# TSultanov/cfd-demo

Hardware: AMD Instinct MI355X
Metric: cell-updates/s (Poisson iter) + ms/timestep, 4096² grid, 1/2/4/8 GPU (higher is better)
Workload: dtype f32

## Files before the change

### cfd-demo_amd/cfdamd/__init__.py

```python
from __future__ import annotations

import ctypes as C
import enum
from dataclasses import dataclass
from typing import List, Optional

import numpy as np

from . import _lib
from ._lib import (CFD_ENONFINITE, CfdError, CfdGrid, CfdParams, CfdResiduals, CfdState, check,
                   load)

__all__ = [
    "VelocityScheme", "InletProfile", "PressureSolver", "BoundaryKind", "Cylinder", "Grid",
    "SimulationParams", "Residuals", "SimSnapshot", "Model", "SimulationControlHandle",
    "CfdError", "default_grid", "cavity_grid", "rccl_unique_id", "device_count", "load", "LocalHub",
    "VisualizationMode", "CFD_ENONFINITE",
]


class VelocityScheme(enum.IntEnum):
    FirstOrder = 0
    SecondOrder = 1

# ... 385 lines not shown
        return {"state": int(s.value), "m0": int(a.value), "rm": int(b.value)}

    @property
    def comm_calls(self) -> int:
        n = C.c_uint64()
        check("cfd_get_comm_calls", load().cfd_get_comm_calls(self._hh(), C.byref(n)))
        return int(n.value)

    @property
    def recoveries(self) -> int:
        n = C.c_uint64()
        check("cfd_get_recoveries", load().cfd_get_recoveries(self._hh(), C.byref(n)))
        return int(n.value)

    @property
    def resident_solves(self) -> int:
        n = C.c_uint64()
        check("cfd_get_resident_solves", load().cfd_get_resident_solves(self._hh(), C.byref(n)))
        return int(n.value)

    @property
    def persist_blocks(self) -> int:
        n = C.c_int()
        check("cfd_get_persist_blocks", load().cfd_get_persist_blocks(self._hh(), C.byref(n)))
        return n.value

    @property
    def comm_size(self) -> int:
        n = C.c_int()
        check("cfd_get_comm_size", load().cfd_get_comm_size(self._hh(), C.byref(n)))
# ... 107 lines not shown
```

### cfd-demo_amd/cfdamd/_lib.py

```python
from __future__ import annotations

import ctypes as C
import os

PKG_DIR = os.path.dirname(os.path.abspath(__file__))
ROOT = os.path.dirname(PKG_DIR)
LIB_PATH = os.environ.get("CFD_LIB") or os.path.join(ROOT, "lib", "libcfd_amd.so")

EXPORTS = [
    "cfd_default_params", "cfd_default_grid", "cfd_create", "cfd_rccl_unique_id",
    "cfd_create_sharded", "cfd_local_hub_create", "cfd_local_hub_destroy",
    "cfd_create_sharded_local", "cfd_device_count", "cfd_get_comm_size", "cfd_get_slab", "cfd_update", "cfd_update_n", "cfd_piso_step",
    "cfd_pressure_solve", "cfd_run_phase", "cfd_set_params", "cfd_get_snapshot",
    "cfd_get_residuals", "cfd_get_state", "cfd_set_state", "cfd_get_masks", "cfd_synchronize",
    "cfd_profile_sweeps", "cfd_timing_begin", "cfd_timing_end", "cfd_timing_phases",
    "cfd_timing_phase_ms", "cfd_timing_exchange_ms", "cfd_get_halo_depth",
    "cfd_get_kernel_config", "cfd_get_jacobi_kernel", "cfd_get_persist_blocks", "cfd_get_persist_steals", "cfd_get_persist_sums", "cfd_get_sums_launches", "cfd_get_sums_bounds", "cfd_get_recoveries", "cfd_get_comm_calls", "cfd_get_resident_solves", "cfd_get_jacobi_geometry", "cfd_plan_slab", "cfd_plan_sweep", "cfd_plan_halo", "cfd_plan_block", "cfd_plan_overlap",
    "cfd_render", "cfd_derive_field", "cfd_last_error", "cfd_abi_version", "cfd_destroy",
    "cfd_get_config", "cfd_run_start", "cfd_run_stop", "cfd_run_pause", "cfd_run_resume",
    "cfd_run_set_params", "cfd_run_request_snapshot", "cfd_run_last_snapshot",
    "cfd_run_new_residuals", "cfd_run_status", "cfd_run_steps",
    "cfd_polygon_new", "cfd_polygon_new_rect", "cfd_polygon_new_regular", "cfd_polygon_add_hole",
    "cfd_polygon_contains_point", "cfd_polygon_intersects_aabb",
    "cfd_polygon_edges_intersect_aabb", "cfd_polygon_bounding_box",
    "cfd_polygon_bounding_square", "cfd_polygon_edges", "cfd_polygon_destroy",
    "cfd_geom_do_intersect", "cfd_geom_segment_intersection", "cfd_geom_intersect_quad_edge",
    "cfd_tesselate", "cfd_quadtree_size", "cfd_quadtree_nodes", "cfd_quadtree_destroy",
    "cfd_mesh_from_quadtree", "cfd_mesh_sizes", "cfd_mesh_cells", "cfd_mesh_neighbors",
    "cfd_mesh_intersections", "cfd_mesh_full_bounding_box", "cfd_mesh_build_ms",
    "cfd_mesh_destroy",
]

# ... 93 lines not shown
        "cfd_timing_phases": (i32, [vp, i32]),
        "cfd_timing_phase_ms": (i32, [vp, C.POINTER(C.c_double), C.POINTER(C.c_double)]),
        "cfd_timing_exchange_ms": (i32, [vp, C.POINTER(C.c_double), C.POINTER(C.c_uint64)]),
        "cfd_get_halo_depth": (i32, [vp]),
        "cfd_get_kernel_config": (i32, [vp, C.POINTER(i32), C.POINTER(i32)]),
        "cfd_get_jacobi_kernel": (i32, [vp, C.POINTER(i32), C.c_char_p, C.c_size_t]),
        "cfd_get_persist_blocks": (i32, [vp, C.POINTER(i32)]),
        "cfd_get_persist_steals": (i32, [vp, C.POINTER(C.c_uint64)]),
        "cfd_get_persist_sums": (i32, [vp, C.POINTER(C.c_uint64)]),
        "cfd_get_sums_launches": (i32, [vp, C.POINTER(C.c_uint64)]),
        "cfd_get_sums_bounds": (i32, [vp, C.POINTER(C.c_uint32), C.POINTER(C.c_uint32),
                                      C.POINTER(C.c_uint32)]),
        "cfd_get_recoveries": (i32, [vp, C.POINTER(C.c_uint64)]),
        "cfd_get_comm_calls": (i32, [vp, C.POINTER(C.c_uint64)]),
        "cfd_get_resident_solves": (i32, [vp, C.POINTER(C.c_uint64)]),
        "cfd_get_jacobi_geometry": (i32, [vp, i32, C.POINTER(i32), C.POINTER(i32), C.POINTER(i32),
                                          C.POINTER(i32)]),
        "cfd_plan_slab": (i32, [C.c_uint64, i32, i32, C.POINTER(C.c_uint64),
                                C.POINTER(C.c_uint64)]),
        "cfd_plan_sweep": (i32, [i32, i32, i32, i32, i32, i32, C.POINTER(i32), C.POINTER(i32),
                                 C.POINTER(i32)]),
        "cfd_plan_halo": (i32, [i32, i32, i32, i32, i32, C.POINTER(i32)]),
        "cfd_plan_overlap": (i32, [i32, i32, i32, i32, i32, i32, C.POINTER(i32)]),
        "cfd_plan_block": (i32, [i32, i32, i32, i32, i32, i32, i32, C.POINTER(i32),
                                 C.POINTER(i32), C.POINTER(i32), C.POINTER(i32)]),
        "cfd_render": (i32, [vp, i32, C.POINTER(C.c_uint8), FP]),
        "cfd_derive_field": (i32, [vp, i32, FP, FP]),
        "cfd_last_error": (C.c_char_p, []),
        "cfd_abi_version": (i32, []),
        "cfd_destroy": (None, [vp]),
# ... 57 lines not shown
```

### cfd-demo_amd/csrc/cfd_device.h

```cpp
#pragma once
#include "cfd_internal.h"

#include <algorithm>

namespace cfd {
namespace {

inline int cdiv(long a, long b) { return (int)((a + b - 1) / b); }


constexpr int kBlock = 256;
typedef unsigned int u32x4 __attribute__((ext_vector_type(4)));

__device__ __forceinline__ float dt_of(const Ctl *c, float dt_override) {
    return __builtin_isnan(dt_override) ? c->dt : dt_override;
}

__device__ __forceinline__ bool pass_off(const Ctl *c, int pass) {
    return pass >= 0 && c->go[pass] == 0;
}

__device__ __forceinline__ float wave_max(float m) {
#pragma unroll
    for (int o = 32; o > 0; o >>= 1) m = fmaxf(m, __shfl_xor(m, o, 64));
// ... 58 lines not shown
}

template <int SP>
__device__ __forceinline__ float sdiv(float x, float c, float r) {
    return SP ? x * r : x / c;
}

typedef float f2 __attribute__((ext_vector_type(2)));

template <int FAST>
__device__ __forceinline__ f2 fdiv2(f2 x, float c, float r) {
    if (FAST == 1) return x * r;
    return (f2){fdiv<FAST>(x.x, c, r), fdiv<FAST>(x.y, c, r)};
}

__device__ __forceinline__ void solve_finalize_body(const Geom &g, const Fields &f, int pass,
                                                    int iters, int check_break, int flips,
                                                    int exact_flips) {
    Ctl *c = f.ctl;
    __shared__ int go_s;
    const int k_lo = g.tol_enabled ? 0 : (iters > 0 ? iters - 1 : 0);
    const int wv = (int)threadIdx.x >> 6, nw = (int)blockDim.x >> 6;
    for (int k = k_lo + wv; k < iters; k += nw) {
        uint32_t *set = f.err_slots + (size_t)k * kResSlots * kResStride;
        const float v = read_max(set, c->err[k]);
        if ((threadIdx.x & 63) < kResSlots) set[(threadIdx.x & 63) * kResStride] = 0u;
        if ((threadIdx.x & 63) == 0) c->err[k] = __float_as_uint(v);
    }
    __syncthreads();
    if (threadIdx.x == 0) {
        const int go = pass < 0 ? 1 : c->go[pass];
        if (go) {
            int n = iters;
            if (g.tol_enabled && iters > 0) {
                n = 1;
                while (n < iters && !(__uint_as_float(c->err[n - 1]) < g.p_tol)) ++n;
            }
            const float res = n > 0 ? __uint_as_float(c->err[n - 1]) : 0.0f;
            c->cur = (c->cur + (exact_flips == 2 ? c->spec_launches
                                : (g.tol_enabled && !exact_flips) ? n : flips)) & 1;
            c->last_p = res;
            c->red[5] = __float_as_uint(res);
            c->n_exec_last = (uint32_t)n;
            c->sweeps_total += (uint64_t)n;
        }
        if (pass >= 0 && pass + 1 <= kMaxPasses)
            c->go[pass + 1] = (go && !(check_break && g.tol_enabled && c->last_p < g.p_tol)) ? 1 : 0;
        if (exact_flips >= 2) c->spec_stop = c->spec_redo = c->spec_launch = c->spec_launches = 0;
        c->sums_state = 0u;
        c->sums_m0 = 0u;
        go_s = go;
    }
    __syncthreads();
    if (go_s)
        for (int k = threadIdx.x; k < iters; k += blockDim.x) c->err[k] = 0u;
}

template <int FAST>
__device__ __forceinline__ float4 jacobi_row4(const float4 &B, const float4 &C, const float4 &T,
                                              const float4 &Rh, float L0, float R3, float dx_sq,
                                              float dy_sq, float denom, float r_dx_sq,
                                              float r_dy_sq, float r_denom) {
    const f2 c01 = {C.x, C.y}, c23 = {C.z, C.w};
    const f2 h01 = __builtin_shufflevector(c01, c01, 1, 0) + (f2){L0, C.z};
    const f2 h23 = __builtin_shufflevector(c23, c23, 1, 0) + (f2){C.y, R3};
    const f2 v01 = (f2){T.x, T.y} + (f2){B.x, B.y};
    const f2 v23 = (f2){T.z, T.w} + (f2){B.z, B.w};
    const f2 hz01 = fdiv2<FAST>(h01, dx_sq, r_dx_sq), hz23 = fdiv2<FAST>(h23, dx_sq, r_dx_sq);
    const f2 vt01 = fdiv2<FAST>(v01, dy_sq, r_dy_sq), vt23 = fdiv2<FAST>(v23, dy_sq, r_dy_sq);
    const f2 pu01 = fdiv2<FAST>(hz01 + vt01 - (f2){Rh.x, Rh.y}, denom, r_denom);
// ... 11 lines not shown
```

### cfd-demo_amd/csrc/cfd_internal.h

```cpp
#pragma once
#include <hip/hip_runtime.h>
#include <stdint.h>

#include "../../include/cfd.h"

namespace cfd {

constexpr int kGhostUV = 2;
constexpr float kSumsPLim = 0x1p122f, kSumsRLim = 0x1p112f;
constexpr int kMaxSweeps = 4096;
constexpr int kMaxPasses = 64;

constexpr int kResSlots = 32;
constexpr int kResStride = 16;
constexpr int kPersistFlagStride = 16;
constexpr int kPersistHeadLines = 21;
constexpr int kPersistBlockBits = 10;
static_assert((1 << kPersistBlockBits) > kMaxSweeps / 8, "persistent flag layout");
constexpr int kPersistMaxGroups = 16384;
constexpr size_t kPersistWords = (size_t)(kPersistMaxGroups + kPersistHeadLines) * kPersistFlagStride;
constexpr size_t kSlotWords = (size_t)(kMaxSweeps + 16) * kResSlots * kResStride + kPersistWords;

struct Ctl {
    float dt;
// ... 2 lines not shown
    float inlet;
    int32_t cur;
    uint32_t n_exec_last;
    float last_p;
    float res_u, res_v;
    uint32_t red[7];
    uint32_t nonfinite_step;
    uint32_t vis[2];
    uint32_t sums_state;
    uint64_t sweeps_total;
    int32_t spec_stop, spec_redo, spec_launch, spec_launches;
    uint32_t sums_launches;
    uint32_t sums_m0, sums_rm;
    int32_t go[kMaxPasses + 1];
    uint32_t err[kMaxSweeps];
};

struct Geom {
    int32_t nx, ny;
    int32_t j0, nyl;
    int32_t hg;
    float dx, dy, nu, ly;
    float target_inlet;
    int32_t scheme, profile, bc_kind;
    int32_t tol_enabled;
    float p_tol;
    int32_t jacobi_iters;
    float dx_sq, dy_sq, denom;
    float r_dx_sq, r_dy_sq, r_denom;
    int32_t fastdiv;
    int32_t tb_rows;
// ... 30 lines not shown
void launch_step_begin(const Geom &g, const Fields &f, int copy, hipStream_t s);
void launch_copy_star(const Geom &g, const Fields &f, int pass, hipStream_t s);
void launch_copy_star_div(const Geom &g, const Fields &f, int pass, float dt_override,
                          hipStream_t s);
void launch_u_predictor(const Geom &g, const Fields &f, float dt_override, hipStream_t s);
void launch_v_predictor(const Geom &g, const Fields &f, float dt_override, hipStream_t s);
void launch_predict(const Geom &g, const Fields &f, float dt_override, hipStream_t s);
bool predict_march_ok(const Geom &g, const Fields &f);
void launch_predict_march(const Geom &g, const Fields &f, float dt_override, hipStream_t s,
                          bool set_inlet = false, int row_lo = 0, int row_hi = -1);
void launch_divergence(const Geom &g, const Fields &f, int pass, float dt_override,
                       hipStream_t s);
void launch_jacobi_sweep(const Geom &g, const Fields &f, int pass, int it, int row_lo,
                         int row_hi, int res, hipStream_t s);
void launch_jacobi_block(const Geom &g, const Fields &f, int pass, int it, int par, int T,
                         int out_lo, int out_hi, int res, hipStream_t s);
bool launch_jacobi_persist(const Geom &g, const Fields &f, int pass, int par0, int nblk,
                           int out_lo, int out_hi, uint32_t epoch, int res_it, hipStream_t s);
void lds_geometry8(const Geom &g, int out_lo, int out_hi, bool persist, int *pad, int *occ, int *nwc,
                   int *nseg);
void launch_tb1(const Geom &g, const Fields &f, int T, int pass, int it, int par, int out_lo,
                int out_hi, uint32_t *res_slots, hipStream_t s);
void launch_pipe(const Geom &g, const Fields &f, int T, int pass, int it, int par, int out_lo,
                 int out_hi, uint32_t *res_slots, hipStream_t s);
bool launch_lds_persist8(const Geom &g, const Fields &f, int pass, int par0, int nblk, int out_lo,
                         int out_hi, uint32_t epoch, uint32_t *rs, hipStream_t s);
void launch_lds(const Geom &g, const Fields &f, int T, int pass, int it, int par, int out_lo,
                int out_hi, uint32_t *res_slots, hipStream_t s, int mode = 0, int lag = 0);
void launch_jacobi_spec(const Geom &g, const Fields &f, int pass, int it, int par, int T,
                        int out_lo, int out_hi, hipStream_t s, int lag = 0);
void launch_spec_check(const Geom &g, const Fields &f, int pass, int it, int T, int par,
// ... 45 lines not shown
void launch_mg_prolong_smooth5(const MgLevel &Cl, const float *e, const MgLevel &L, const float *src,
                               float *dst, const Ctl *ctl, int pass, hipStream_t s);
void launch_mg_smooth5_residual(const MgLevel &L, const float *src, float *dst, const Ctl *ctl,
                                int pass, hipStream_t s);
void launch_mg_residual(const MgLevel &L, const float *p, const Ctl *ctl, int pass, hipStream_t s);
void launch_mg_restrict(const MgLevel &F, const MgLevel &Cl, const Ctl *ctl, int pass, hipStream_t s);
void launch_mg_prolong_add(const MgLevel &Cl, const float *e, const MgLevel &F, float *p,
                           const Ctl *ctl, int pass, hipStream_t s);
void launch_mg_tail(const MgLevel *dev_levels, int s_level, int coarsest, float *a0, float *b0,
                    int fast, const Ctl *ctl, int pass, hipStream_t s);
void launch_mg_final_residual(const MgLevel &L, const float *p, uint32_t *slots, const Ctl *ctl,
                              int pass, hipStream_t s);
void launch_corrector(const Geom &g, const Fields &f, int pass, float dt_override,
                      hipStream_t s);
void launch_boundary(const Geom &g, const Fields &f, hipStream_t s);
void launch_correct_finish(const Geom &g, const Fields &f, float dt_override, hipStream_t s);
void launch_step_reduce(const Geom &g, const Fields &f, hipStream_t s);
void launch_publish_sums_m0(const Geom &g, const Fields &f, hipStream_t s);
bool correct_head_ok(const Geom &g, const Fields &f);
void launch_correct_head(const Geom &g, const Fields &f, int pass, float dt_override, bool has_next,
                         hipStream_t s);
void launch_step_finalize(const Geom &g, const Fields &f, hipStream_t s);
void launch_abort_to_red(const Fields &f, hipStream_t s);
void launch_abort_from_red(const Fields &f, hipStream_t s);

constexpr int kJacRowsPerWave = 16;
constexpr int kMaxTemporal = 8;
constexpr int kJacWavesPerBlock = 4;

}
```

### cfd-demo_amd/csrc/cfd_jacobi_lds.h

```cpp
#pragma once
#include <cmath>
#include <type_traits>

#include "cfd_device.h"

namespace cfd {
namespace {

constexpr int kLdsWaves = 4;
#ifndef CFD_LDS_SB
#define CFD_LDS_SB 0
#endif
#ifndef CFD_LDS_PD
#define CFD_LDS_PD 3
#endif
#ifndef CFD_LDS_DIAG
#define CFD_LDS_DIAG 0
#endif
#ifndef CFD_LDS_WPE
#define CFD_LDS_WPE 0
#endif
typedef unsigned int u32x2 __attribute__((ext_vector_type(2)));
#ifndef CFD_LDS_PRIO
#define CFD_LDS_PRIO 1
// ... 427 lines not shown
            ctl->spec_launch = lpar;
            ctl->spec_redo = j + 1 < T ? j + 1 : 0;
        }
    }
    return j;
}

template <int T, int FAST, int MODE>
__global__ __launch_bounds__(kLdsWaves * 64, lds_min_waves(MODE)) void k_jacobi_lds(
    Geom g, float *__restrict__ pa, float *__restrict__ pb, const float *__restrict__ rhs,
    Ctl *ctl, uint32_t *res_slots, int pass, int par, int out_lo, int out_hi, int nwc, int nseg,
    int wlo, int whi, int it, int lag, float sums_c) {
    using M = LdsMarch<T, FAST, MODE>;
    [[maybe_unused]] constexpr bool RES = M::RES;
    __shared__ f2 lds[kLdsWaves * M::D * 64];
#if CFD_LDS_STAMP
    const unsigned long long st_rt0 = __builtin_amdgcn_s_memrealtime();
    const unsigned long long st_t0 = __builtin_amdgcn_s_memtime();
    struct StampOnExit {
        unsigned long long rt0, t0;
        unsigned long long bid;
        __device__ ~StampOnExit() {
            if (RES) return;
            const unsigned long long rt1 = __builtin_amdgcn_s_memrealtime();
            const unsigned long long t1 = __builtin_amdgcn_s_memtime();
            const unsigned hw = __builtin_amdgcn_s_getreg(4 | (31 << 11));
            const unsigned xcc = __builtin_amdgcn_s_getreg(20 | (31 << 11));
            const int idx = (int)blockIdx.x * kLdsWaves + ((int)threadIdx.x >> 6);
            if ((threadIdx.x & 63) == 0 && idx < kStampWaves) {
                g_lds_stamp[idx * 4 + 0] = rt0;
                g_lds_stamp[idx * 4 + 1] = rt1;
                g_lds_stamp[idx * 4 + 2] = (bid << 40) | ((t1 - t0) & 0xFFFFFFFFFFull);
                g_lds_stamp[idx * 4 + 3] = ((unsigned long long)xcc << 32) | hw;
            }
        }
    } stamp_guard{st_rt0, st_t0, (unsigned long long)xcd_block(g)};
#endif
    if (pass_off(ctl, pass)) return;
    int nst = 0;
    if constexpr (M::SPEC) {
        if (lag > 0) {
            __shared__ int stop_s;
            if (threadIdx.x == 0) stop_s = ctl->spec_stop;
            __syncthreads();
            if (stop_s) return;
            if (spec_lag_first(g, ctl, res_slots - (size_t)lag * kResSlots * kResStride, it - lag, lag,
                               par - 1) < lag)
                return;
        } else if (ctl->spec_stop) {
            return;
        }
    }
    if constexpr (M::REDO) {
// ... 1 lines not shown
            const int j = spec_lag_first(g, ctl, res_slots, it, lag, par, false);
            nst = j + 1 < lag ? j + 1 : 0;
        } else {
            nst = ctl->spec_redo;
            par = ctl->spec_launch;
        }
        if (nst <= 0) return;
    }
    if constexpr (FAST == 1 && MODE <= 1) {
        if (sums_c > 0.0f && ctl->sums_state == 2u) {
            const float bound = __uint_as_float(ctl->sums_m0) * g.r_dx_sq + sums_c * __uint_as_float(ctl->sums_rm);
            if (bound < 0x1p123f) {
                if (blockIdx.x == 0 && threadIdx.x == 0) atomicAdd(&ctl->sums_launches, 1u);
                lds_block<T, FAST, MODE, 2>(g, pa, pb, rhs, ctl, res_slots, par, out_lo, out_hi, nwc, nseg,
                                            wlo, whi, lds, nst, xcd_block(g));
                return;
            }
        }
    }
    lds_block<T, FAST, MODE>(g, pa, pb, rhs, ctl, res_slots, par, out_lo, out_hi, nwc, nseg, wlo,
                             whi, lds, nst, xcd_block(g));
}

constexpr int kStealDepth = 16;
#ifndef CFD_PERSIST_WPE
#define CFD_PERSIST_WPE 3
#endif
template <int T, int FAST>
__global__ __launch_bounds__(kLdsWaves * 64, CFD_PERSIST_WPE) void k_jacobi_persist(
    Geom g, float *__restrict__ pa, float *__restrict__ pb, const float *__restrict__ rhs,
    Ctl *ctl, uint32_t *persist, uint32_t *host_fail, uint32_t *res_slots, uint32_t epoch, int pass,
    int par0, int nblk, int out_lo, int out_hi, int nwc, int nseg, int wlo, int whi, int ngrp,
    int acq, uint32_t deadline, uint32_t steal, int late, int sums, float plim, float rlim) {
    using M = LdsMarch<T, FAST, 4>;
    __shared__ f2 lds[kLdsWaves * M::D * 64];
    __shared__ int run_tile_s, run_blk_s, abort_s, own_next_s, sp_s, fast_s;
// ... 297 lines not shown

template <int T>
void launch_lds_T(const Geom &g, const Fields &f, int pass, int par, int it, int out_lo, int out_hi,
                  uint32_t *rs, int mode, hipStream_t s, int lag = 0) {
    if (mode == 2) {
        launch_lds_t<T, 2>(g, f, pass, par, it, out_lo, out_hi, rs, s, lag);
        return;
    }
    if constexpr (T == 8) {
        if (mode == 3) {
            launch_lds_t<8, 3>(g, f, pass, par, it, out_lo, out_hi, rs, s, lag);
            return;
        }
    }
    if (rs)
        launch_lds_t<T, 1>(g, f, pass, par, it, out_lo, out_hi, rs, s);
    else
        launch_lds_t<T, 0>(g, f, pass, par, it, out_lo, out_hi, rs, s);
}

template <int T, int FAST>
int persist_blocks_per_cu(int pad) {
    static int cache[2] = {0, 0};
    int &nb = cache[pad > 0 ? 1 : 0];
    if (nb == 0) {
        int n = 0;
        if (hipOccupancyMaxActiveBlocksPerMultiprocessor(
                &n, reinterpret_cast<const void *>(&k_jacobi_persist<T, FAST>), kLdsWaves * 64, pad) !=
                hipSuccess ||
            n < 1)
            n = 1;
// ... 66 lines not shown
```

### cfd-demo_amd/csrc/cfd_kernels.hip

```cpp
#include "cfd_device.h"
#include "cfd_predict.h"

namespace cfd {

typedef float f4u __attribute__((ext_vector_type(4), aligned(4)));

namespace {
__global__ __launch_bounds__(kBlock) void k_verify_division(float c, float r,
                                                            unsigned long long *counts) {
    const uint32_t tid = blockIdx.x * blockDim.x + threadIdx.x;
    const uint32_t stride = gridDim.x * blockDim.x;
    uint32_t bad1 = 0, bad2 = 0, bad3 = 0;
    for (uint64_t k = tid; k < (1ull << 32); k += stride) {
        const float x = __uint_as_float((uint32_t)k);
        const float ref = x / c;
        const float m1 = fdiv<1>(x, c, r);
        const float m2 = fdiv<2>(x, c, r);
        const float m3 = fdiv<3>(x, c, r);
        const bool rn = ref != ref;
        bad1 += (rn ? (m1 == m1) : (__float_as_uint(m1) != __float_as_uint(ref))) ? 1u : 0u;
        bad2 += (rn ? (m2 == m2) : (__float_as_uint(m2) != __float_as_uint(ref))) ? 1u : 0u;
        bad3 += (rn ? (m3 == m3) : (__float_as_uint(m3) != __float_as_uint(ref))) ? 1u : 0u;
    }
#pragma unroll
// ... 921 lines not shown
        float4 p = *reinterpret_cast<const float4 *>(f.p + rp);
        p.x = p.x + pc.x;
        p.y = p.y + pc.y;
        p.z = p.z + pc.z;
        p.w = p.w + pc.w;
        *reinterpret_cast<float4 *>(f.p + rp) = p;
    }
}

#ifndef CFD_CF_ROWS
#define CFD_CF_ROWS 16
#endif
constexpr int kCfRows = CFD_CF_ROWS;
template <int SP, int ROWS>
__global__ __launch_bounds__(kBlock) void k_correct_finish4m(Geom g, Fields f, float dt_override,
                                                             int nbx) {
    Ctl *c = f.ctl;
    const int nx = g.nx;
    float du = 0.f, dv = 0.f, mu = 0.f, mv = 0.f;
    uint32_t pm = 0u;
    bool bad = false;
    const int bid = xcd_block(g);
    const int i0 = 4 * ((bid % nbx) * kBlock + (int)threadIdx.x);
    const int l0 = (bid / nbx) * ROWS, l1 = min(l0 + ROWS, g.nyl + 1);
    const float dt = dt_of(c, dt_override);
    const float inlet = c->inlet;
    const float *__restrict__ pp = c->cur ? f.pp[1] : f.pp[0];
    if (i0 < nx) {
        float4 pb = make_float4(0.f, 0.f, 0.f, 0.f);
        {
            const int j = g.j0 + l0;
// ... 28 lines not shown
    mv = wave_max(mv);
    const int wv = threadIdx.x >> 6;
    if ((threadIdx.x & 63) == 0) {
        red[wv][0] = du;
        red[wv][1] = dv;
        red[wv][2] = mu;
        red[wv][3] = mv;
    }
    __syncthreads();
    if (threadIdx.x < 4) {
        float r = 0.f;
#pragma unroll
        for (int w = 0; w < kBlock / 64; ++w) r = fmaxf(r, red[w][threadIdx.x]);
        publish_max(f.red_slots + (size_t)threadIdx.x * kResSlots * kResStride, bid, r);
    }
}


__global__ __launch_bounds__(kBlock) void k_step_reduce(Geom g, Fields f) {
    const size_t tid = blockIdx.x * (size_t)blockDim.x + threadIdx.x;
    const size_t stride = (size_t)gridDim.x * blockDim.x;
    const size_t nu = (size_t)g.nyl * (g.nx + 1), nv = (size_t)(g.nyl + 1) * g.nx;
    float du = 0.f, dv = 0.f, mu = 0.f, mv = 0.f;
    bool bad = false;
    for (size_t k = tid; k < nu; k += stride) {
        const float a = f.u[k];
        du = fmaxf(du, fabsf(a - f.u_old[k]));
        mu = fmaxf(mu, fabsf(a));
        bad |= nonfinite(a);
    }
// ... 135 lines not shown
    const int nseg = cdiv(row_hi - row_lo, kJacRowsPerWave);
    float *pa = f.pp[0] - (long)g.hg * g.nx, *pb = f.pp[1] - (long)g.hg * g.nx;
    const dim3 grid(nbx * nseg), block(kJacWavesPerBlock * 64);
    if (g.fastdiv == 1)
        hipLaunchKernelGGL((k_jacobi<kJacRowsPerWave, 1>), grid, block, 0, s, g, pa, pb, f.rhs,
                           f.ctl, f.err_slots, pass, it, row_lo, row_hi, nbx, res);
    else if (g.fastdiv == 2)
        hipLaunchKernelGGL((k_jacobi<kJacRowsPerWave, 2>), grid, block, 0, s, g, pa, pb, f.rhs,
                           f.ctl, f.err_slots, pass, it, row_lo, row_hi, nbx, res);
    else
        hipLaunchKernelGGL((k_jacobi<kJacRowsPerWave, 0>), grid, block, 0, s, g, pa, pb, f.rhs,
                           f.ctl, f.err_slots, pass, it, row_lo, row_hi, nbx, res);
}

void launch_jacobi_block(const Geom &g, const Fields &f, int pass, int it, int par, int T,
                         int out_lo, int out_hi, int res, hipStream_t s) {
    if (out_hi <= out_lo) return;
    uint32_t *rs = res ? f.err_slots + (size_t)(it + T - 1) * kResSlots * kResStride : nullptr;
    if (g.tb_kind == 4)
        launch_pipe(g, f, T, pass, it, par, out_lo, out_hi, rs, s);
    else if (g.tb_kind == 5)
        launch_lds(g, f, T, pass, it, par, out_lo, out_hi, rs, s);
    else
        launch_tb1(g, f, T, pass, it, par, out_lo, out_hi, rs, s);
}

bool launch_jacobi_persist(const Geom &g, const Fields &f, int pass, int par0, int nblk,
                           int out_lo, int out_hi, uint32_t epoch, int res_it, hipStream_t s) {
    if (out_hi <= out_lo || nblk < 1 || g.tb_kind != 5 || !f.persist) return false;
    uint32_t *rs = res_it >= 0 ? f.err_slots + (size_t)res_it * kResSlots * kResStride : nullptr;
    return launch_lds_persist8(g, f, pass, par0, nblk, out_lo, out_hi, epoch, rs, s);
}

void launch_jacobi_spec(const Geom &g, const Fields &f, int pass, int it, int par, int T,
                        int out_lo, int out_hi, hipStream_t s, int lag) {
    if (out_hi <= out_lo) return;
    launch_lds(g, f, T, pass, it, par, out_lo, out_hi,
// ... 73 lines not shown
    const int hn = has_next ? 1 : 0;
    const int nrows = g.nyl + 1 + 2 * kGhostUV;
    const int rows = cf_rows(g, nbx4, nrows);
    const dim3 grid(nbx4 * cdiv(nrows, rows));
#define CFD_LAUNCH_CH(SPV, RW)                                                                    \
    hipLaunchKernelGGL((k_correct_head4<SPV, RW>), grid, dim3(kBlock), 0, s, g, f, pass, dt_override, \
                       nbx4, hn)
    if (rows == kCfRows) {
        if (g.sp_pow2) CFD_LAUNCH_CH(1, kCfRows); else CFD_LAUNCH_CH(0, kCfRows);
    } else {
        if (g.sp_pow2) CFD_LAUNCH_CH(1, 1); else CFD_LAUNCH_CH(0, 1);
    }
#undef CFD_LAUNCH_CH
}

void launch_correct_finish(const Geom &g, const Fields &f, float dt_override, hipStream_t s) {
    auto a16 = [](const void *p) { return ((uintptr_t)p & 15u) == 0; };
    if (g.nx % 4 == 0 && a16(f.pp[0]) && a16(f.pp[1]) && a16(f.p) && a16(f.v) && a16(f.v_star)) {
        const int nbx = cdiv(g.nx / 4, kBlock);
        const int rows = cf_rows(g, nbx, g.nyl + 1);
        const dim3 grid(nbx * cdiv(g.nyl + 1, rows));
#define CFD_LAUNCH_CF(SPV, RW)                                                                     \
    hipLaunchKernelGGL((k_correct_finish4m<SPV, RW>), grid, dim3(kBlock), 0, s, g, f, dt_override, nbx)
        if (rows == kCfRows) {
            if (g.sp_pow2) CFD_LAUNCH_CF(1, kCfRows); else CFD_LAUNCH_CF(0, kCfRows);
        } else {
            if (g.sp_pow2) CFD_LAUNCH_CF(1, 1); else CFD_LAUNCH_CF(0, 1);
        }
#undef CFD_LAUNCH_CF
        return;
    }
    const int nbx = cdiv(g.nx + 1, kBlock);
    const long ntiles = (long)nbx * (g.nyl + 1);
    const int blocks = (int)std::min<long>(ntiles, 8L * g.n_cu);
    if (g.sp_pow2)
        hipLaunchKernelGGL(k_correct_finish<1>, dim3(blocks), dim3(kBlock), 0, s, g, f, dt_override, nbx);
    else
        hipLaunchKernelGGL(k_correct_finish<0>, dim3(blocks), dim3(kBlock), 0, s, g, f, dt_override, nbx);
}

void launch_boundary(const Geom &g, const Fields &f, hipStream_t s) {
    hipLaunchKernelGGL(k_boundary, dim3(1), dim3(1024), 0, s, g, f);
}

void launch_step_reduce(const Geom &g, const Fields &f, hipStream_t s) {
    const size_t n = (size_t)(g.nyl + 1) * (g.nx + 1);
    hipLaunchKernelGGL(k_step_reduce, dim3(copy_grid(n / 4 + 1)), dim3(kBlock), 0, s, g, f);
}

void launch_publish_sums_m0(const Geom &g, const Fields &f, hipStream_t s) {
    const size_t n = (size_t)g.nx * (size_t)g.nyl;
    hipLaunchKernelGGL(k_publish_sums_m0, dim3(copy_grid(n)), dim3(kBlock), 0, s, g, f);
}
// ... 15 lines not shown
```

### cfd-demo_amd/csrc/cfd_model.hip

```cpp
#include <hip/hip_runtime.h>
#include <rccl/rccl.h>

#include <chrono>
#include <cmath>
#include <initializer_list>
#include <condition_variable>
#include <memory>
#include <mutex>
#include <thread>
#include <cstdio>
#include <cstring>
#include <string>
#include <functional>
#include <vector>

#include "../../include/cfd.h"
#include "cfd_internal.h"
#include "slab_plan.h"

using namespace cfd;

namespace {

thread_local std::string g_last_error;
// ... 939 lines not shown
        if (params.pressure_solver == CFD_SOLVER_SOR) return enqueue_sor(pass);
        if (params.pressure_solver == CFD_SOLVER_MULTIGRID) return enqueue_mg(pass);
        const int iters = params.jacobi_iters;
        const int lo_g = 1 - (int)j0, hi_g = (int)g.ny - 1 - (int)j0;
        bool evt = timing && pass <= 0;
        hipEvent_t e0 = nullptr, e1 = nullptr;
        if (evt) {
            e0 = take_event();
            e1 = take_event();
            HIP_TRY(hipEventRecord(e0, stream));
        }
        const bool spec = spec_mode();
        const int tmax = g.tol_enabled ? 1 : t_max;
        int launches = 0;
        bool resident = false;
        if (!sharded()) {
            if (spec && resident_mode() && !capturing) {
                PersistGate &gate = persist_gate(device);
                std::lock_guard<std::mutex> lk(gate.mu);
                if (gate.last && gate.last != stream) {
                    hipStreamCaptureStatus cs = hipStreamCaptureStatusNone;
                    (void)hipStreamIsCapturing(gate.last, &cs);
                    if (cs == hipStreamCaptureStatusNone) {
                        if (!gate.ev) HIP_TRY(hipEventCreateWithFlags(&gate.ev, hipEventDisableTiming));
                        HIP_TRY(hipEventRecord(gate.ev, gate.last));
                        HIP_TRY(hipStreamWaitEvent(stream, gate.ev, 0));
                    }
                }
                resident = launch_jacobi_resident(g, f, pass, iters, 1, pass >= 1 ? 1 : 0, stream);
                if (resident) {
// ... 43 lines not shown
                        k += T;
                        ++nblk;
                    }
                    bool done = false;
                    int rc = launch_persist(pass, launches, nblk, lo_g, hi_g, res_it, &done);
                    if (rc) return rc;
                    if (done) {
                        last_persist_blocks = nblk;
                        it = 8 * nblk;
                        launches = nblk;
                    }
                }
                for (; it < iters;) {
                    int T, lo, hi, exch;
                    plan_block((int)j0, g.nyl, g.ny, 0, it, tmax, iters, &T, &lo, &hi, &exch);
                    launch_jacobi_block(g, f, pass, it, launches, T, lo, hi, it + T == iters,
                                        stream);
                    it += T;
                    ++launches;
                }
            }
            if (evt) HIP_TRY(hipEventRecord(e1, stream));
        } else if (g.tol_enabled && spec_slab_ok()) {
            const int n = enqueue_spec_slabs(pass, evt ? e1 : nullptr);
            if (n < 0) return n;
            if (evt) {
                solve_events.emplace_back(e0, e1);
                timed_sweeps += (uint64_t)iters;
                timed_launches += (uint64_t)n;
            }
            return 0;
        } else {
// ... 85 lines not shown
                ++launches;
                if (exch && !ovl) {
                    int rc = exchange_pp((host_cur + launches) & 1, g.hg);
                    if (rc) return rc;
                }
            }
            const int last = iters > 0 ? iters - 1 : 0;
            if (!merge_res_allreduce) {
                launch_fold_slots(f.ctl->err + last,
                                  f.err_slots + (size_t)last * kResSlots * kResStride, 1, stream);
                int rc = allreduce_max_u32(f.ctl->err + last, 1);
                if (rc) return rc;
            }
            if (evt) HIP_TRY(hipEventRecord(e1, stream));
        }
        if (resident) {
        } else {
            launch_finalize_solve(g, f, pass, iters, pass >= 1 ? 1 : 0, launches, stream,
                                  spec ? 2 : 0);
        }
        HIP_TRY(hipGetLastError());
        if (evt) {
            solve_events.emplace_back(e0, e1);
            timed_sweeps += (uint64_t)iters;
            timed_launches += (uint64_t)launches;
        }
        host_cur = (host_cur + launches) & 1;
        return 0;
    }

    int enqueue_solve_host_driven(float *residual_out) {
        if (params.pressure_solver == CFD_SOLVER_SOR) {
            hipEvent_t e0;
            begin_solve_timing(-1, &e0);
// ... 204 lines not shown
            launch_predict_march(g, f, dt_override, stream, true, 2, g.nyl - 2);
            HIP_TRY(hipStreamWaitEvent(stream, ev_uv, 0));
            launch_predict_march(g, f, dt_override, stream, false, 0, 4);
            launch_predict_march(g, f, dt_override, stream, false, g.nyl - 4, g.nyl);
        } else if (march)
            launch_predict_march(g, f, dt_override, stream, finish && step_begin_folded);
        else
            launch_predict(g, f, dt_override, stream);
        auto first_divergence = [&](int pass) {
            if (!march) launch_divergence(g, f, pass, dt_override, stream);
            phase_mark(0, true);
        };
        if (finish) {
            first_divergence(host_driven() ? -1 : 0);
            merge_res_allreduce = sharded() && !host_driven();
            int rc = host_driven() ? enqueue_solve_host_driven(nullptr) : enqueue_solve(0);
            merge_res_allreduce = false;
            if (rc) return rc;
            phase_mark(1, false);
            launch_correct_finish(g, f, dt_override, stream);
            phase_mark(1, true);
            HIP_TRY(hipGetLastError());
            return 0;
        }
        if (!host_driven()) {
            first_divergence(0);
            int rc = enqueue_solve(0);
            if (rc) return rc;
            const int passes = params.corrector_passes;
            const bool fuse = !sharded() && passes >= 1 && correct_head_ok(g, f);
            auto corrector = [&](int pass) {
                if (fuse)
                    launch_correct_head(g, f, pass, dt_override, pass < passes, stream);
                else
                    launch_corrector(g, f, pass, dt_override, stream);
// ... 17 lines not shown
                pass_head(-1, dt_override);
                rc = enqueue_solve_host_driven(&res);
                if (rc) return rc;
                launch_corrector(g, f, -1, dt_override, stream);
                if (res < params.p_tol) break;
            }
        }
        launch_boundary(g, f, stream);
        HIP_TRY(hipGetLastError());
        return 0;
    }

    bool step_begin_folded = false;
    bool merge_res_allreduce = false;
    bool uv_async = false;
    int enqueue_update(bool rec_step = true) {
        if (rec_step) HIP_TRY(hipEventRecord(ev_step0, stream));
        const bool fused = params.corrector_passes == 0;
        step_begin_folded = fused && predict_march_ok(g, f);
        if (!step_begin_folded) launch_step_begin(g, f, fused ? 0 : 1, stream);
        uv_async = sharded() && overlap && fused && step_begin_folded && g.nyl >= 8;
        int rc;
        if (uv_async) {
            HIP_TRY(hipEventRecord(ev_ov0, stream));
            HIP_TRY(hipStreamWaitEvent(cstream, ev_ov0, 0));
            rc = exchange_uv(cstream);
            if (rc) return rc;
            HIP_TRY(hipEventRecord(ev_uv, cstream));
        } else {
            rc = exchange_uv();
        }
        if (rc) return rc;
        rc = enqueue_piso(kNaN, fused);
        if (rc) return rc;
        if (!fused) launch_step_reduce(g, f, stream);
        if (!fused && f.sums_track) launch_publish_sums_m0(g, f, stream);
        if (sharded()) launch_fold_slots(f.ctl->red, f.red_slots, 4, stream);
        if (sharded() && persist_env && persist_sharded_env) launch_abort_to_red(f, stream);
        rc = allreduce_max_u32(f.ctl->red, 7);
        if (rc) return rc;
        launch_step_finalize(g, f, stream);
        HIP_TRY(hipGetLastError());
        if (rec_step) HIP_TRY(hipEventRecord(ev_step1, stream));
        if (timing) timed_steps++;
        if (rec_step) stepped = true;
        return 0;
    }
    std::vector<hipEvent_t> step_events;

    hipGraphExec_t step_graph = nullptr;
    int graph_cur_delta = 0;
    int graph_steps = 4;
    bool graph_enabled = [] {
        const char *e = getenv("CFD_GRAPH");
        return e && atoi(e) != 0;
    }();
// ... 1235 lines not shown
    return 0;
}

int cfd_get_comm_calls(const cfd_model *m, uint64_t *n) {
    if (!m || !n) return fail(CFD_EINVAL, "null argument");
    *n = m->comm_calls;
    return 0;
}

int cfd_get_recoveries(const cfd_model *m, uint64_t *n) {
    if (!m || !n) return fail(CFD_EINVAL, "null argument");
    *n = m->recoveries;
    return 0;
}

int cfd_get_resident_solves(const cfd_model *m, uint64_t *solves) {
    if (!m || !solves) return fail(CFD_EINVAL, "null argument");
    *solves = m->resident_solves;
    return 0;
}

int cfd_get_persist_blocks(const cfd_model *m, int *blocks) {
    if (!m || !blocks) return fail(CFD_EINVAL, "null argument");
    *blocks = m->last_persist_blocks;
    return 0;
}

int cfd_plan_slab(uint64_t ny, int n_ranks, int rank, uint64_t *j0, uint64_t *j1) {
    if (n_ranks < 1 || rank < 0 || rank >= n_ranks || !j0 || !j1)
        return fail(CFD_EINVAL, "bad plan_slab arguments");
// ... 38 lines not shown
```

### include/cfd.h

```cpp
#ifndef CFD_H
#define CFD_H

#include <stddef.h>
#include <stdint.h>

#ifdef __cplusplus
extern "C" {
#endif

#define CFD_ABI_VERSION 1

typedef enum {
    CFD_OK = 0,
    CFD_EINVAL = -1,
    CFD_EHIP = -2,
    CFD_ERCCL = -3,
    CFD_ESTATE = -4,
    CFD_ENONFINITE = -5,
    CFD_ETIMEOUT = -6,
} cfd_status;

typedef struct cfd_model cfd_model;

typedef struct {
// ... 86 lines not shown
                   uint64_t *steps);
int cfd_timing_phases(cfd_model *m, int on);
int cfd_timing_phase_ms(const cfd_model *m, double *predict_ms, double *finish_ms);
int cfd_timing_exchange_ms(const cfd_model *m, double *exchange_ms, uint64_t *exchanges);
int cfd_get_halo_depth(const cfd_model *m);
int cfd_get_kernel_config(const cfd_model *m, int *fastdiv, int *temporal);
int cfd_get_jacobi_kernel(const cfd_model *m, int *kind, char *name, size_t name_len);

int cfd_get_persist_blocks(const cfd_model *m, int *blocks);
int cfd_get_persist_steals(cfd_model *m, uint64_t *steals);
int cfd_get_persist_sums(cfd_model *m, uint64_t *blocks);
int cfd_get_sums_launches(cfd_model *m, uint64_t *launches);
int cfd_get_sums_bounds(cfd_model *m, uint32_t *state, uint32_t *m0_bits, uint32_t *rm_bits);
int cfd_get_comm_calls(const cfd_model *m, uint64_t *n);
int cfd_get_recoveries(const cfd_model *m, uint64_t *n);
int cfd_get_resident_solves(const cfd_model *m, uint64_t *solves);
int cfd_get_jacobi_geometry(const cfd_model *m, int persist, int *lds_pad, int *wgs_per_cu,
                            int *wave_cols, int *segments);

int cfd_plan_slab(uint64_t ny, int n_ranks, int rank, uint64_t *j0, uint64_t *j1);
int cfd_plan_sweep(int j0, int nyl, int ny, int halo_depth, int it, int iters, int *lo, int *hi,
                   int *exchange);
int cfd_plan_halo(int kind, int nyl, int depth, int rank, int n_ranks, int *out6);
int cfd_plan_overlap(int nyl, int halo_depth, int rank, int n_ranks, int lo, int hi, int *out6);
int cfd_plan_block(int j0, int nyl, int ny, int halo_depth, int it, int t_max, int iters, int *T,
                   int *out_lo, int *out_hi, int *exchange);

typedef enum { CFD_VIS_PRESSURE = 0, CFD_VIS_VELOCITY = 1, CFD_VIS_VORTICITY = 2 } cfd_vis_mode;

int cfd_render(cfd_model *m, int mode, uint8_t *rgba, float *min_max_out);
// ... 71 lines not shown
```

Before: 2944 billion.

## Fold solve and step finalize into last workgroup of preceding kernels

```diff
diff --git a/cfd-demo_amd/cfdamd/__init__.py b/cfd-demo_amd/cfdamd/__init__.py
--- a/cfd-demo_amd/cfdamd/__init__.py
+++ b/cfd-demo_amd/cfdamd/__init__.py
@@ -423,6 +423,13 @@
         return int(n.value)
 
     @property
+    def finalize_launches(self) -> dict:
+        a, b = C.c_uint64(), C.c_uint64()
+        check("cfd_get_finalize_launches",
+              load().cfd_get_finalize_launches(self._hh(), C.byref(a), C.byref(b)))
+        return {"solve": int(a.value), "step": int(b.value)}
+
+    @property
     def resident_solves(self) -> int:
         n = C.c_uint64()
         check("cfd_get_resident_solves", load().cfd_get_resident_solves(self._hh(), C.byref(n)))
diff --git a/cfd-demo_amd/cfdamd/_lib.py b/cfd-demo_amd/cfdamd/_lib.py
--- a/cfd-demo_amd/cfdamd/_lib.py
+++ b/cfd-demo_amd/cfdamd/_lib.py
@@ -15,7 +15,7 @@
     "cfd_get_residuals", "cfd_get_state", "cfd_set_state", "cfd_get_masks", "cfd_synchronize",
     "cfd_profile_sweeps", "cfd_timing_begin", "cfd_timing_end", "cfd_timing_phases",
     "cfd_timing_phase_ms", "cfd_timing_exchange_ms", "cfd_get_halo_depth",
-    "cfd_get_kernel_config", "cfd_get_jacobi_kernel", "cfd_get_persist_blocks", "cfd_get_persist_steals", "cfd_get_persist_sums", "cfd_get_sums_launches", "cfd_get_sums_bounds", "cfd_get_recoveries", "cfd_get_comm_calls", "cfd_get_resident_solves", "cfd_get_jacobi_geometry", "cfd_plan_slab", "cfd_plan_sweep", "cfd_plan_halo", "cfd_plan_block", "cfd_plan_overlap",
+    "cfd_get_kernel_config", "cfd_get_jacobi_kernel", "cfd_get_persist_blocks", "cfd_get_persist_steals", "cfd_get_persist_sums", "cfd_get_sums_launches", "cfd_get_sums_bounds", "cfd_get_recoveries", "cfd_get_comm_calls", "cfd_get_resident_solves", "cfd_get_finalize_launches", "cfd_get_jacobi_geometry", "cfd_plan_slab", "cfd_plan_sweep", "cfd_plan_halo", "cfd_plan_block", "cfd_plan_overlap",
     "cfd_render", "cfd_derive_field", "cfd_last_error", "cfd_abi_version", "cfd_destroy",
     "cfd_get_config", "cfd_run_start", "cfd_run_stop", "cfd_run_pause", "cfd_run_resume",
     "cfd_run_set_params", "cfd_run_request_snapshot", "cfd_run_last_snapshot",
@@ -139,6 +139,7 @@
         "cfd_get_recoveries": (i32, [vp, C.POINTER(C.c_uint64)]),
         "cfd_get_comm_calls": (i32, [vp, C.POINTER(C.c_uint64)]),
         "cfd_get_resident_solves": (i32, [vp, C.POINTER(C.c_uint64)]),
+        "cfd_get_finalize_launches": (i32, [vp, C.POINTER(C.c_uint64), C.POINTER(C.c_uint64)]),
         "cfd_get_jacobi_geometry": (i32, [vp, i32, C.POINTER(i32), C.POINTER(i32), C.POINTER(i32),
                                           C.POINTER(i32)]),
         "cfd_plan_slab": (i32, [C.c_uint64, i32, i32, C.POINTER(C.c_uint64),
diff --git a/cfd-demo_amd/csrc/cfd_device.h b/cfd-demo_amd/csrc/cfd_device.h
--- a/cfd-demo_amd/csrc/cfd_device.h
+++ b/cfd-demo_amd/csrc/cfd_device.h
@@ -96,15 +96,14 @@
     return (f2){fdiv<FAST>(x.x, c, r), fdiv<FAST>(x.y, c, r)};
 }
 
-__device__ __forceinline__ void solve_finalize_body(const Geom &g, const Fields &f, int pass,
-                                                    int iters, int check_break, int flips,
-                                                    int exact_flips) {
-    Ctl *c = f.ctl;
-    __shared__ int go_s;
-    const int k_lo = g.tol_enabled ? 0 : (iters > 0 ? iters - 1 : 0);
+__device__ __forceinline__ void solve_finalize_work(int tol_enabled, float p_tol, Ctl *c,
+                                                    uint32_t *err_slots, int pass, int iters,
+                                                    int check_break, int flips, int exact_flips,
+                                                    int *go_s) {
+    const int k_lo = tol_enabled ? 0 : (iters > 0 ? iters - 1 : 0);
     const int wv = (int)threadIdx.x >> 6, nw = (int)blockDim.x >> 6;
     for (int k = k_lo + wv; k < iters; k += nw) {
-        uint32_t *set = f.err_slots + (size_t)k * kResSlots * kResStride;
+        uint32_t *set = err_slots + (size_t)k * kResSlots * kResStride;
         const float v = read_max(set, c->err[k]);
         if ((threadIdx.x & 63) < kResSlots) set[(threadIdx.x & 63) * kResStride] = 0u;
         if ((threadIdx.x & 63) == 0) c->err[k] = __float_as_uint(v);
@@ -114,28 +113,52 @@
         const int go = pass < 0 ? 1 : c->go[pass];
         if (go) {
             int n = iters;
-            if (g.tol_enabled && iters > 0) {
+            if (tol_enabled && iters > 0) {
                 n = 1;
-                while (n < iters && !(__uint_as_float(c->err[n - 1]) < g.p_tol)) ++n;
+                while (n < iters && !(__uint_as_float(c->err[n - 1]) < p_tol)) ++n;
             }
             const float res = n > 0 ? __uint_as_float(c->err[n - 1]) : 0.0f;
             c->cur = (c->cur + (exact_flips == 2 ? c->spec_launches
-                                : (g.tol_enabled && !exact_flips) ? n : flips)) & 1;
+                                : (tol_enabled && !exact_flips) ? n : flips)) & 1;
             c->last_p = res;
             c->red[5] = __float_as_uint(res);
             c->n_exec_last = (uint32_t)n;
             c->sweeps_total += (uint64_t)n;
         }
         if (pass >= 0 && pass + 1 <= kMaxPasses)
-            c->go[pass + 1] = (go && !(check_break && g.tol_enabled && c->last_p < g.p_tol)) ? 1 : 0;
+            c->go[pass + 1] = (go && !(check_break && tol_enabled && c->last_p < p_tol)) ? 1 : 0;
         if (exact_flips >= 2) c->spec_stop = c->spec_redo = c->spec_launch = c->spec_launches = 0;
         c->sums_state = 0u;
         c->sums_m0 = 0u;
-        go_s = go;
+        *go_s = go;
     }
     __syncthreads();
-    if (go_s)
+    if (*go_s)
         for (int k = threadIdx.x; k < iters; k += blockDim.x) c->err[k] = 0u;
+}
+
+__device__ __forceinline__ void solve_finalize_body(const Geom &g, const Fields &f, int pass,
+                                                    int iters, int check_break, int flips,
+                                                    int exact_flips) {
+    __shared__ int go_s;
+    solve_finalize_work(g.tol_enabled, g.p_tol, f.ctl, f.err_slots, pass, iters, check_break, flips, exact_flips, &go_s);
+}
+
+__device__ __forceinline__ bool last_workgroup_out(uint32_t *ticket, int *flag_s) {
+    asm volatile("s_waitcnt vmcnt(0)" ::: "memory");
+    __syncthreads();
+    if (threadIdx.x == 0) {
+        const bool last = __hip_atomic_fetch_add(ticket, 1u, __ATOMIC_RELAXED, __HIP_MEMORY_SCOPE_AGENT) ==
+                          (uint32_t)gridDim.x - 1u;
+        if (last) {
+            __hip_atomic_store(ticket, 0u, __ATOMIC_RELAXED, __HIP_MEMORY_SCOPE_AGENT);
+            __builtin_amdgcn_fence(__ATOMIC_ACQUIRE, "agent");
+            asm volatile("s_waitcnt vmcnt(0)" ::: "memory");
+        }
+        *flag_s = last;
+    }
+    __syncthreads();
+    return *flag_s != 0;
 }
 
 template <int FAST>
diff --git a/cfd-demo_amd/csrc/cfd_internal.h b/cfd-demo_amd/csrc/cfd_internal.h
--- a/cfd-demo_amd/csrc/cfd_internal.h
+++ b/cfd-demo_amd/csrc/cfd_internal.h
@@ -40,7 +40,9 @@
     uint32_t sums_m0, sums_rm;
     int32_t go[kMaxPasses + 1];
     uint32_t err[kMaxSweeps];
+    uint32_t fold_ticket[2 * 32];
 };
+constexpr int kFoldTicketStride = 32;
 
 struct Geom {
     int32_t nx, ny;
@@ -101,7 +103,7 @@
 void launch_jacobi_sweep(const Geom &g, const Fields &f, int pass, int it, int row_lo,
                          int row_hi, int res, hipStream_t s);
 void launch_jacobi_block(const Geom &g, const Fields &f, int pass, int it, int par, int T,
-                         int out_lo, int out_hi, int res, hipStream_t s);
+                         int out_lo, int out_hi, int res, hipStream_t s, int fin = 0);
 bool launch_jacobi_persist(const Geom &g, const Fields &f, int pass, int par0, int nblk,
                            int out_lo, int out_hi, uint32_t epoch, int res_it, hipStream_t s);
 void lds_geometry8(const Geom &g, int out_lo, int out_hi, bool persist, int *pad, int *occ, int *nwc,
@@ -177,7 +179,8 @@
 void launch_corrector(const Geom &g, const Fields &f, int pass, float dt_override,
                       hipStream_t s);
 void launch_boundary(const Geom &g, const Fields &f, hipStream_t s);
-void launch_correct_finish(const Geom &g, const Fields &f, float dt_override, hipStream_t s);
+bool launch_correct_finish(const Geom &g, const Fields &f, float dt_override, hipStream_t s,
+                           bool fold_step = false);
 void launch_step_reduce(const Geom &g, const Fields &f, hipStream_t s);
 void launch_publish_sums_m0(const Geom &g, const Fields &f, hipStream_t s);
 bool correct_head_ok(const Geom &g, const Fields &f);
diff --git a/cfd-demo_amd/csrc/cfd_jacobi_lds.h b/cfd-demo_amd/csrc/cfd_jacobi_lds.h
--- a/cfd-demo_amd/csrc/cfd_jacobi_lds.h
+++ b/cfd-demo_amd/csrc/cfd_jacobi_lds.h
@@ -465,6 +465,17 @@
     using M = LdsMarch<T, FAST, MODE>;
     [[maybe_unused]] constexpr bool RES = M::RES;
     __shared__ f2 lds[kLdsWaves * M::D * 64];
+    [[maybe_unused]] const int tol_enabled = g.tol_enabled;
+    [[maybe_unused]] const float p_tol = g.p_tol;
+    auto fold = [&]() {
+        if constexpr (MODE == 1) {
+            if (lag == 0) return;
+            int *words = reinterpret_cast<int *>(lds);
+            if (!last_workgroup_out(ctl->fold_ticket, words)) return;
+            uint32_t *err_slots = res_slots - (size_t)(it + T - 1) * kResSlots * kResStride;
+            solve_finalize_work(tol_enabled, p_tol, ctl, err_slots, pass, it + T, 0, par + 1, 0, words + 1);
+        }
+    };
 #if CFD_LDS_STAMP
     const unsigned long long st_rt0 = __builtin_amdgcn_s_memrealtime();
     const unsigned long long st_t0 = __builtin_amdgcn_s_memtime();
@@ -487,7 +498,10 @@
         }
     } stamp_guard{st_rt0, st_t0, (unsigned long long)xcd_block(g)};
 #endif
-    if (pass_off(ctl, pass)) return;
+    if (pass_off(ctl, pass)) {
+        fold();
+        return;
+    }
     int nst = 0;
     if constexpr (M::SPEC) {
         if (lag > 0) {
@@ -519,12 +533,14 @@
                 if (blockIdx.x == 0 && threadIdx.x == 0) atomicAdd(&ctl->sums_launches, 1u);
                 lds_block<T, FAST, MODE, 2>(g, pa, pb, rhs, ctl, res_slots, par, out_lo, out_hi, nwc, nseg,
                                             wlo, whi, lds, nst, xcd_block(g));
+                fold();
                 return;
             }
         }
     }
     lds_block<T, FAST, MODE>(g, pa, pb, rhs, ctl, res_slots, par, out_lo, out_hi, nwc, nseg, wlo,
                              whi, lds, nst, xcd_block(g));
+    fold();
 }
 
 constexpr int kStealDepth = 16;
@@ -852,7 +868,7 @@
         }
     }
     if (rs)
-        launch_lds_t<T, 1>(g, f, pass, par, it, out_lo, out_hi, rs, s);
+        launch_lds_t<T, 1>(g, f, pass, par, it, out_lo, out_hi, rs, s, lag);
     else
         launch_lds_t<T, 0>(g, f, pass, par, it, out_lo, out_hi, rs, s);
 }
diff --git a/cfd-demo_amd/csrc/cfd_kernels.hip b/cfd-demo_amd/csrc/cfd_kernels.hip
--- a/cfd-demo_amd/csrc/cfd_kernels.hip
+++ b/cfd-demo_amd/csrc/cfd_kernels.hip
@@ -959,7 +959,7 @@
 constexpr int kCfRows = CFD_CF_ROWS;
 template <int SP, int ROWS>
 __global__ __launch_bounds__(kBlock) void k_correct_finish4m(Geom g, Fields f, float dt_override,
-                                                             int nbx) {
+                                                             int nbx, int fold) {
     Ctl *c = f.ctl;
     const int nx = g.nx;
     float du = 0.f, dv = 0.f, mu = 0.f, mv = 0.f;
@@ -1018,6 +1018,9 @@
         for (int w = 0; w < kBlock / 64; ++w) r = fmaxf(r, red[w][threadIdx.x]);
         publish_max(f.red_slots + (size_t)threadIdx.x * kResSlots * kResStride, bid, r);
     }
+    if (!fold) return;
+    __shared__ int last_s;
+    if (last_workgroup_out(c->fold_ticket + kFoldTicketStride, &last_s)) step_finalize_body(g, f);
 }
 
 
@@ -1183,13 +1186,13 @@
 }
 
 void launch_jacobi_block(const Geom &g, const Fields &f, int pass, int it, int par, int T,
-                         int out_lo, int out_hi, int res, hipStream_t s) {
+                         int out_lo, int out_hi, int res, hipStream_t s, int fin) {
     if (out_hi <= out_lo) return;
     uint32_t *rs = res ? f.err_slots + (size_t)(it + T - 1) * kResSlots * kResStride : nullptr;
     if (g.tb_kind == 4)
         launch_pipe(g, f, T, pass, it, par, out_lo, out_hi, rs, s);
     else if (g.tb_kind == 5)
-        launch_lds(g, f, T, pass, it, par, out_lo, out_hi, rs, s);
+        launch_lds(g, f, T, pass, it, par, out_lo, out_hi, rs, s, 0, rs && fin ? 1 : 0);
     else
         launch_tb1(g, f, T, pass, it, par, out_lo, out_hi, rs, s);
 }
@@ -1293,21 +1296,23 @@
 #undef CFD_LAUNCH_CH
 }
 
-void launch_correct_finish(const Geom &g, const Fields &f, float dt_override, hipStream_t s) {
+bool launch_correct_finish(const Geom &g, const Fields &f, float dt_override, hipStream_t s,
+                           bool fold_step) {
     auto a16 = [](const void *p) { return ((uintptr_t)p & 15u) == 0; };
     if (g.nx % 4 == 0 && a16(f.pp[0]) && a16(f.pp[1]) && a16(f.p) && a16(f.v) && a16(f.v_star)) {
         const int nbx = cdiv(g.nx / 4, kBlock);
         const int rows = cf_rows(g, nbx, g.nyl + 1);
         const dim3 grid(nbx * cdiv(g.nyl + 1, rows));
 #define CFD_LAUNCH_CF(SPV, RW)                                                                     \
-    hipLaunchKernelGGL((k_correct_finish4m<SPV, RW>), grid, dim3(kBlock), 0, s, g, f, dt_override, nbx)
+    hipLaunchKernelGGL((k_correct_finish4m<SPV, RW>), grid, dim3(kBlock), 0, s, g, f, dt_override, nbx, \
+                       fold_step ? 1 : 0)
         if (rows == kCfRows) {
             if (g.sp_pow2) CFD_LAUNCH_CF(1, kCfRows); else CFD_LAUNCH_CF(0, kCfRows);
         } else {
             if (g.sp_pow2) CFD_LAUNCH_CF(1, 1); else CFD_LAUNCH_CF(0, 1);
         }
 #undef CFD_LAUNCH_CF
-        return;
+        return fold_step;
     }
     const int nbx = cdiv(g.nx + 1, kBlock);
     const long ntiles = (long)nbx * (g.nyl + 1);
@@ -1316,6 +1321,7 @@
         hipLaunchKernelGGL(k_correct_finish<1>, dim3(blocks), dim3(kBlock), 0, s, g, f, dt_override, nbx);
     else
         hipLaunchKernelGGL(k_correct_finish<0>, dim3(blocks), dim3(kBlock), 0, s, g, f, dt_override, nbx);
+    return false;
 }
 
 void launch_boundary(const Geom &g, const Fields &f, hipStream_t s) {
diff --git a/cfd-demo_amd/csrc/cfd_model.hip b/cfd-demo_amd/csrc/cfd_model.hip
--- a/cfd-demo_amd/csrc/cfd_model.hip
+++ b/cfd-demo_amd/csrc/cfd_model.hip
@@ -977,6 +977,7 @@
         const int tmax = g.tol_enabled ? 1 : t_max;
         int launches = 0;
         bool resident = false;
+        bool folded = false;
         if (!sharded()) {
             if (spec && resident_mode() && !capturing) {
                 PersistGate &gate = persist_gate(device);
@@ -1050,8 +1051,10 @@
                 for (; it < iters;) {
                     int T, lo, hi, exch;
                     plan_block((int)j0, g.nyl, g.ny, 0, it, tmax, iters, &T, &lo, &hi, &exch);
+                    const bool fin = fold_solve && pass == 0 && g.tb_kind == 5 && it + T == iters && hi > lo;
                     launch_jacobi_block(g, f, pass, it, launches, T, lo, hi, it + T == iters,
-                                        stream);
+                                        stream, fin);
+                    folded = folded || fin;
                     it += T;
                     ++launches;
                 }
@@ -1167,10 +1170,11 @@
             }
             if (evt) HIP_TRY(hipEventRecord(e1, stream));
         }
-        if (resident) {
+        if (resident || folded) {
         } else {
             launch_finalize_solve(g, f, pass, iters, pass >= 1 ? 1 : 0, launches, stream,
                                   spec ? 2 : 0);
+            ++finalize_solve_launches;
         }
         HIP_TRY(hipGetLastError());
         if (evt) {
@@ -1405,11 +1409,13 @@
         if (finish) {
             first_divergence(host_driven() ? -1 : 0);
             merge_res_allreduce = sharded() && !host_driven();
+            fold_solve = step_fold();
             int rc = host_driven() ? enqueue_solve_host_driven(nullptr) : enqueue_solve(0);
             merge_res_allreduce = false;
+            fold_solve = false;
             if (rc) return rc;
             phase_mark(1, false);
-            launch_correct_finish(g, f, dt_override, stream);
+            step_finalize_folded = launch_correct_finish(g, f, dt_override, stream, fold_step);
             phase_mark(1, true);
             HIP_TRY(hipGetLastError());
             return 0;
@@ -1457,6 +1463,18 @@
     bool step_begin_folded = false;
     bool merge_res_allreduce = false;
     bool uv_async = false;
+    bool step_fold_env = [] {
+        const char *e = getenv("CFD_STEP_FOLD");
+        return !(e && atoi(e) == 0);
+    }();
+    bool step_fold() const {
+        return step_fold_env && !sharded() && !g.tol_enabled &&
+               params.pressure_solver == CFD_SOLVER_JACOBI;
+    }
+    uint64_t finalize_solve_launches = 0, step_finalize_launches = 0;
+    bool fold_solve = false;
+    bool fold_step = false;
+    bool step_finalize_folded = false;
     int enqueue_update(bool rec_step = true) {
         if (rec_step) HIP_TRY(hipEventRecord(ev_step0, stream));
         const bool fused = params.corrector_passes == 0;
@@ -1474,7 +1492,10 @@
             rc = exchange_uv();
         }
         if (rc) return rc;
+        fold_step = fused && step_fold();
+        step_finalize_folded = false;
         rc = enqueue_piso(kNaN, fused);
+        fold_step = false;
         if (rc) return rc;
         if (!fused) launch_step_reduce(g, f, stream);
         if (!fused && f.sums_track) launch_publish_sums_m0(g, f, stream);
@@ -1482,7 +1503,10 @@
         if (sharded() && persist_env && persist_sharded_env) launch_abort_to_red(f, stream);
         rc = allreduce_max_u32(f.ctl->red, 7);
         if (rc) return rc;
-        launch_step_finalize(g, f, stream);
+        if (!step_finalize_folded) {
+            launch_step_finalize(g, f, stream);
+            ++step_finalize_launches;
+        }
         HIP_TRY(hipGetLastError());
         if (rec_step) HIP_TRY(hipEventRecord(ev_step1, stream));
         if (timing) timed_steps++;
@@ -2748,6 +2772,13 @@
     return 0;
 }
 
+int cfd_get_finalize_launches(const cfd_model *m, uint64_t *solve, uint64_t *step) {
+    if (!m || !solve || !step) return fail(CFD_EINVAL, "null argument");
+    *solve = m->finalize_solve_launches;
+    *step = m->step_finalize_launches;
+    return 0;
+}
+
 int cfd_get_resident_solves(const cfd_model *m, uint64_t *solves) {
     if (!m || !solves) return fail(CFD_EINVAL, "null argument");
     *solves = m->resident_solves;
diff --git a/include/cfd.h b/include/cfd.h
--- a/include/cfd.h
+++ b/include/cfd.h
@@ -124,6 +124,7 @@
 int cfd_get_sums_bounds(cfd_model *m, uint32_t *state, uint32_t *m0_bits, uint32_t *rm_bits);
 int cfd_get_comm_calls(const cfd_model *m, uint64_t *n);
 int cfd_get_recoveries(const cfd_model *m, uint64_t *n);
+int cfd_get_finalize_launches(const cfd_model *m, uint64_t *solve, uint64_t *step);
 int cfd_get_resident_solves(const cfd_model *m, uint64_t *solves);
 int cfd_get_jacobi_geometry(const cfd_model *m, int persist, int *lds_pad, int *wgs_per_cu,
                             int *wave_cols, int *segments);
```

Result: no change. 2961 billion (median of 6 runs) (+0.6%).
